# GuanLab/seekmer

Measured on AMD Instinct MI355X. Metric: paired reads/sec mapped+quantified, higher is better.
Workload: dtype u64+f64; 1 GPU; configs[1]: synthetic ~190k-tx index (stand-in for ENSEMBL GRCh38 cDNA), 10000000 2x100bp synthetic pairs per GPU, map+classes+EM to the reference stop rule; transcripts=190402, kmer_slots=134217728, units_per_gpu=10000000, read_len=100, paired=True, classes=851072, class_map_rows=4208693, parallelism=reads sharded x1, RCCL all-reduce f64[T] per EM step, rccl_ranks=0

## Files before the change

include/seekmer_hip.h:

```cpp
#ifndef SEEKMER_HIP_H
#define SEEKMER_HIP_H

#include <stddef.h>
#include <stdint.h>

#ifdef __cplusplus
extern "C" {
#endif

#define SKM_OK 0
#define SKM_ERR_ARG 1
#define SKM_ERR_HIP 2
#define SKM_ERR_NO_DEVICE 3
#define SKM_ERR_COLLISION 4
#define SKM_ERR_STATE 5
#define SKM_ERR_IO 6
#define SKM_ERR_UNDEFINED 7
#define SKM_ERR_COMM 8

#define SKM_KMER_SIZE 25
#define SKM_MAX_FRAGMENT_LENGTH 2000


const char *skm_last_error(void);
// ... 16 lines not shown
                     const char *sequences, int64_t n_bases,
                     const void *targets, int64_t n_targets,
                     int device, skm_index **out);
int skm_index_destroy(skm_index *index);
int skm_index_info(const skm_index *index, int64_t info[8]);
int skm_index_layout(const skm_index *index, int64_t layout[8]);
int skm_index_junctions(const skm_index *index, int32_t *succ, uint8_t *kept);
int skm_index_probe(const skm_index *index, int mode, const uint64_t *kmers, int64_t n, int32_t *entry,
                    int32_t *offset);
int skm_index_build_transcripts(skm_index *index, const double *lengths, int64_t n_tx);
int skm_index_transcript_bases(skm_index *index, char *bases_out, uint8_t *known_out);

typedef struct skm_mapper skm_mapper;
int skm_mapper_create(skm_index *index, skm_mapper **out);
int skm_mapper_destroy(skm_mapper *mapper);

int skm_mapper_map_batch(skm_mapper *mapper, const char *bases,
                         const int64_t *offsets, int64_t n_units, int paired);
int skm_mapper_map_batch_async(skm_mapper *mapper, const char *bases,
                               const int64_t *offsets, int64_t n_units, int paired,
                               int64_t first_unit);
int skm_mapper_map_batch_uniform_async(skm_mapper *mapper, const char *bases, int32_t read_len,
                                       int64_t n_units, int paired, int64_t first_unit);
int skm_mapper_sync(skm_mapper *mapper);
int skm_mapper_expect_units(skm_mapper *mapper, int64_t n_units);
#define SKM_PACKED_CUT (-1)
typedef struct skm_packed_reads {
    int32_t stream;
    int32_t code_words;
    int64_t first_read;
    int64_t n_reads;
    int64_t read_stride;
    int64_t uniform_len;
    const uint64_t *codes;
    const uint32_t *lengths;
    int64_t n_exceptions;
    const uint32_t *exception_reads;
    const uint32_t *exception_masks;
    const char *names;
    const int64_t *name_offsets;
} skm_packed_reads;
int skm_mapper_push_packed(skm_mapper *mapper, const skm_packed_reads *piece, int paired);
typedef int (*skm_packed_source)(void *context, skm_packed_reads *piece);
int skm_mapper_map_packed_source(skm_mapper *mapper, skm_packed_source next, void *context,
                                 int paired, int64_t *n_pieces);
int skm_mapper_map_batch_device(skm_mapper *mapper, const void *d_bases,
                                const void *d_offsets, int64_t n_units,
                                int paired, int32_t max_read_len);
int skm_mapper_last_batch(skm_mapper *mapper, int32_t *begin, int32_t *end,
                          int32_t *anchor_entry, int32_t *anchor_offset,
                          int32_t *counts, int32_t *entries,
                          int64_t cap_entries, int64_t *n_entries);
int skm_mapper_keep_spans(skm_mapper *mapper, int enable);
#define SKM_STRAND_NONE 0
#define SKM_STRAND_FR 1
#define SKM_STRAND_RF 2
int skm_mapper_set_strand(skm_mapper *mapper, int mode);
int skm_mapper_set_length_weights(skm_mapper *mapper, const double *p);
int skm_mapper_set_bias(skm_mapper *mapper, int enable);
int skm_mapper_bias_observed(skm_mapper *mapper, int64_t out[4096]);
int skm_mapper_summary(skm_mapper *mapper, int64_t summary[4]);
int skm_mapper_export(skm_mapper *mapper, int64_t *class_offsets,
                      int32_t *class_targets, int64_t *class_counts,
                      int64_t *first_seen, int64_t *fld);
int skm_mapper_merge(skm_mapper *mapper, int64_t n_classes,
                     const int64_t *class_offsets, const int32_t *class_targets,
                     const int64_t *class_counts, const int64_t *first_seen,
                     int64_t unaligned, const int64_t *fld);
typedef struct skm_device_table {
    int32_t device;
    int64_t n_classes, n_ids;
    const int64_t *class_start;
    const int64_t *class_len;
    const double *class_count;
    const uint64_t *first_seen;
    const int32_t *ids;
    int64_t unaligned, units, first_seen_bound;
    const uint64_t *fld;
} skm_device_table;
int skm_mapper_device_table(skm_mapper *mapper, skm_device_table *out);
int skm_mapper_merge_device(skm_mapper *mapper, const skm_device_table *table);
int skm_mapper_clear(skm_mapper *mapper);
int skm_mapper_reset(skm_mapper *mapper);
int skm_mapper_timing(skm_mapper *mapper, double stats[8]);
int skm_mapper_map_relaunches(skm_mapper *mapper, int64_t *count);
int skm_mapper_set_stats(skm_mapper *mapper, int enable);
int skm_mapper_access_stats(skm_mapper *mapper, int64_t out[48]);

typedef struct skm_sample_set skm_sample_set;
int skm_sample_set_create(skm_index *index, int paired, skm_sample_set **out);
int skm_sample_set_destroy(skm_sample_set *set);
int skm_sample_set_set_strand(skm_sample_set *set, int mode);
int skm_sample_set_set_length_weights(skm_sample_set *set, const double *p);
int skm_sample_set_add_packed(skm_sample_set *set, int64_t sample, int64_t first_unit,
                              const skm_packed_reads *mate1, const skm_packed_reads *mate2);
int skm_sample_set_add_batch(skm_sample_set *set, int64_t sample, int64_t first_unit,
                             const char *bases, const int64_t *offsets, int64_t n_units);
int skm_sample_set_sync(skm_sample_set *set);
int skm_sample_set_map_relaunches(skm_sample_set *set, int64_t *count);
int skm_sample_set_summary(skm_sample_set *set, int64_t cap_samples, int64_t *n_samples,
                           int64_t *summary);
int skm_sample_set_export(skm_sample_set *set, int64_t *sample_class_offsets,
                          int64_t *class_offsets, int32_t *class_targets, int64_t *class_counts,
                          int64_t *first_seen);
int skm_sample_set_histogram(skm_sample_set *set, int64_t *fld);
int skm_sample_set_keep_histograms(skm_sample_set *set, int enable);
// ... 192 lines not shown
```

seekmer_amd/_native.py:

```python
import ctypes
import os

_HERE = os.path.dirname(os.path.abspath(__file__))
HIP_LIB_PATH = os.environ.get('SKM_HIP_LIB') or os.path.join(_HERE, 'libseekmer_hip.so')
HOST_LIB_PATH = os.path.join(_HERE, 'libseekmer_host.so')

SKM_OK = 0
SKM_ERR_ARG = 1
SKM_ERR_HIP = 2
SKM_ERR_NO_DEVICE = 3
SKM_ERR_COLLISION = 4
SKM_ERR_STATE = 5
SKM_ERR_IO = 6
SKM_ERR_UNDEFINED = 7
SKM_ERR_COMM = 8

SKM_STRAND_NONE = 0
SKM_STRAND_FR = 1
SKM_STRAND_RF = 2

c_void_pp = ctypes.POINTER(ctypes.c_void_p)
c_i64p = ctypes.POINTER(ctypes.c_int64)
c_i32p = ctypes.POINTER(ctypes.c_int32)
c_f64p = ctypes.POINTER(ctypes.c_double)
# ... 9 lines not shown
                ('exception_reads', ctypes.c_void_p), ('exception_masks', ctypes.c_void_p),
                ('names', ctypes.c_void_p), ('name_offsets', ctypes.c_void_p)]


class DeviceTable(ctypes.Structure):
    _fields_ = [('device', ctypes.c_int32), ('n_classes', ctypes.c_int64), ('n_ids', ctypes.c_int64),
                ('class_start', ctypes.c_void_p), ('class_len', ctypes.c_void_p), ('class_count', ctypes.c_void_p),
                ('first_seen', ctypes.c_void_p), ('ids', ctypes.c_void_p), ('unaligned', ctypes.c_int64),
                ('units', ctypes.c_int64), ('first_seen_bound', ctypes.c_int64), ('fld', ctypes.c_void_p)]


HIP_SYMBOLS = {
    'skm_last_error': (ctypes.c_char_p, []),
    'skm_device_count': (ctypes.c_int, [ctypes.POINTER(ctypes.c_int)]),
    'skm_device_malloc': (ctypes.c_int, [ctypes.c_int, c_i64, c_void_pp]),
    'skm_device_free': (ctypes.c_int, [ctypes.c_int, ctypes.c_void_p]),
    'skm_device_upload': (ctypes.c_int, [ctypes.c_int, ctypes.c_void_p, ctypes.c_void_p, c_i64]),
    'skm_device_download': (ctypes.c_int, [ctypes.c_int, ctypes.c_void_p, ctypes.c_void_p, c_i64]),
    'skm_device_synchronize': (ctypes.c_int, [ctypes.c_int]),
    'skm_device_gather_ceiling': (ctypes.c_int, [ctypes.c_int, c_i64, ctypes.c_int, ctypes.c_int,
                                                 ctypes.c_int, c_f64p]),
    'skm_pinned_alloc': (ctypes.c_void_p, [ctypes.c_size_t]),
    'skm_pinned_free': (None, [ctypes.c_void_p]),
    'skm_pinned_set_device': (ctypes.c_int, [ctypes.c_int]),
    'skm_index_create': (ctypes.c_int, [ctypes.c_void_p, c_i64, ctypes.c_void_p, c_i64,
                                        ctypes.c_void_p, c_i64, ctypes.c_void_p, c_i64,
                                        ctypes.c_int, c_void_pp]),
    'skm_index_destroy': (ctypes.c_int, [ctypes.c_void_p]),
    'skm_index_info': (ctypes.c_int, [ctypes.c_void_p, c_i64p]),
    'skm_index_layout': (ctypes.c_int, [ctypes.c_void_p, c_i64p]),
    'skm_index_junctions': (ctypes.c_int, [ctypes.c_void_p, c_i32p, ctypes.c_void_p]),
    'skm_index_probe': (ctypes.c_int, [ctypes.c_void_p, ctypes.c_int, c_u64p, c_i64, c_i32p, c_i32p]),
    'skm_index_build_transcripts': (ctypes.c_int, [ctypes.c_void_p, c_f64p, c_i64]),
    'skm_index_transcript_bases': (ctypes.c_int, [ctypes.c_void_p, ctypes.c_void_p, ctypes.c_void_p]),
    'skm_mapper_create': (ctypes.c_int, [ctypes.c_void_p, c_void_pp]),
    'skm_mapper_destroy': (ctypes.c_int, [ctypes.c_void_p]),
    'skm_mapper_map_batch': (ctypes.c_int, [ctypes.c_void_p, ctypes.c_void_p, c_i64p, c_i64,
                                            ctypes.c_int]),
    'skm_mapper_map_batch_async': (ctypes.c_int, [ctypes.c_void_p, ctypes.c_void_p, c_i64p, c_i64,
                                                  ctypes.c_int, c_i64]),
    'skm_mapper_map_batch_uniform_async': (ctypes.c_int, [ctypes.c_void_p, ctypes.c_void_p, ctypes.c_int32, c_i64,
                                                          ctypes.c_int, c_i64]),
    'skm_mapper_sync': (ctypes.c_int, [ctypes.c_void_p]),
    'skm_mapper_expect_units': (ctypes.c_int, [ctypes.c_void_p, c_i64]),
    'skm_mapper_push_packed': (ctypes.c_int, [ctypes.c_void_p, ctypes.POINTER(PackedReads), ctypes.c_int]),
    'skm_mapper_map_packed_source': (ctypes.c_int, [ctypes.c_void_p, ctypes.c_void_p, ctypes.c_void_p, ctypes.c_int,
                                                    c_i64p]),
    'skm_mapper_map_batch_device': (ctypes.c_int, [ctypes.c_void_p, ctypes.c_void_p,
                                                   ctypes.c_void_p, c_i64, ctypes.c_int,
                                                   ctypes.c_int32]),
    'skm_mapper_last_batch': (ctypes.c_int, [ctypes.c_void_p, c_i32p, c_i32p, c_i32p, c_i32p,
                                             c_i32p, c_i32p, c_i64, c_i64p]),
    'skm_mapper_keep_spans': (ctypes.c_int, [ctypes.c_void_p, ctypes.c_int]),
    'skm_mapper_set_strand': (ctypes.c_int, [ctypes.c_void_p, ctypes.c_int]),
    'skm_mapper_set_length_weights': (ctypes.c_int, [ctypes.c_void_p, c_f64p]),
    'skm_mapper_set_bias': (ctypes.c_int, [ctypes.c_void_p, ctypes.c_int]),
    'skm_mapper_bias_observed': (ctypes.c_int, [ctypes.c_void_p, c_i64p]),
    'skm_mapper_summary': (ctypes.c_int, [ctypes.c_void_p, c_i64p]),
    'skm_mapper_export': (ctypes.c_int, [ctypes.c_void_p, c_i64p, c_i32p, c_i64p, c_i64p, c_i64p]),
    'skm_mapper_merge': (ctypes.c_int, [ctypes.c_void_p, c_i64, c_i64p, c_i32p, c_i64p, c_i64p,
                                        c_i64, c_i64p]),
    'skm_mapper_device_table': (ctypes.c_int, [ctypes.c_void_p, ctypes.POINTER(DeviceTable)]),
    'skm_mapper_merge_device': (ctypes.c_int, [ctypes.c_void_p, ctypes.POINTER(DeviceTable)]),
    'skm_mapper_clear': (ctypes.c_int, [ctypes.c_void_p]),
    'skm_mapper_reset': (ctypes.c_int, [ctypes.c_void_p]),
    'skm_mapper_timing': (ctypes.c_int, [ctypes.c_void_p, c_f64p]),
    'skm_mapper_map_relaunches': (ctypes.c_int, [ctypes.c_void_p, c_i64p]),
    'skm_sample_set_map_relaunches': (ctypes.c_int, [ctypes.c_void_p, c_i64p]),
    'skm_mapper_set_stats': (ctypes.c_int, [ctypes.c_void_p, ctypes.c_int]),
    'skm_mapper_access_stats': (ctypes.c_int, [ctypes.c_void_p, c_i64p]),
    'skm_effective_lengths': (ctypes.c_int, [ctypes.c_int, c_i64p, c_f64p, c_i64, c_f64p]),
    'skm_effective_lengths_many': (ctypes.c_int, [ctypes.c_int, c_i64, c_i64p, c_f64p, c_i64, c_f64p]),
    'skm_effective_lengths_weights': (ctypes.c_int, [ctypes.c_int, c_i64, c_f64p, c_f64p, c_i64, c_f64p]),
    'skm_bias_correct': (ctypes.c_int, [ctypes.c_void_p, ctypes.c_int, c_i64p, c_f64p, c_f64p, c_i64, c_f64p, c_f64p, c_f64p]),
    'skm_bias_correct_many': (ctypes.c_int, [ctypes.c_void_p, ctypes.c_int, c_i64, c_i64p, c_f64p, c_f64p, c_i64, c_f64p,
                                             c_f64p, c_f64p]),
    'skm_sample_set_create': (ctypes.c_int, [ctypes.c_void_p, ctypes.c_int, c_void_pp]),
    'skm_sample_set_destroy': (ctypes.c_int, [ctypes.c_void_p]),
    'skm_sample_set_set_strand': (ctypes.c_int, [ctypes.c_void_p, ctypes.c_int]),
    'skm_sample_set_set_length_weights': (ctypes.c_int, [ctypes.c_void_p, c_f64p]),
    'skm_sample_set_add_packed': (ctypes.c_int, [ctypes.c_void_p, c_i64, c_i64, ctypes.POINTER(PackedReads),
                                                 ctypes.POINTER(PackedReads)]),
    'skm_sample_set_add_batch': (ctypes.c_int, [ctypes.c_void_p, c_i64, c_i64, ctypes.c_void_p, c_i64p, c_i64]),
    'skm_sample_set_sync': (ctypes.c_int, [ctypes.c_void_p]),
    'skm_sample_set_summary': (ctypes.c_int, [ctypes.c_void_p, c_i64, c_i64p, c_i64p]),
    'skm_sample_set_export': (ctypes.c_int, [ctypes.c_void_p, c_i64p, c_i64p, c_i32p, c_i64p, c_i64p]),
    'skm_sample_set_histogram': (ctypes.c_int, [ctypes.c_void_p, c_i64p]),
    'skm_sample_set_keep_histograms': (ctypes.c_int, [ctypes.c_void_p, ctypes.c_int]),
    'skm_sample_set_histograms': (ctypes.c_int, [ctypes.c_void_p, c_i64, c_i64p]),
    'skm_sample_set_keep_bias': (ctypes.c_int, [ctypes.c_void_p, ctypes.c_int]),
    'skm_sample_set_bias_observed': (ctypes.c_int, [ctypes.c_void_p, c_i64, c_i64p]),
    'skm_sample_set_keep_umis': (ctypes.c_int, [ctypes.c_void_p, ctypes.c_int]),
    'skm_sample_set_add_packed_umis': (ctypes.c_int, [ctypes.c_void_p, c_i64, c_i64, ctypes.POINTER(PackedReads),
                                                      ctypes.POINTER(PackedReads), c_u32p]),
    'skm_sample_set_umi_removed': (ctypes.c_int, [ctypes.c_void_p, c_i64, c_i64p]),
    'skm_umi_windows': (ctypes.c_int, [ctypes.c_int, ctypes.POINTER(PackedReads), ctypes.c_int, ctypes.c_int, c_i32p, c_u32p,
                                       c_i64p]),
    'skm_sample_set_plan': (ctypes.c_int, [c_i64, c_i32p, c_i64p, c_i64, c_i64, c_i64p, c_i64p, c_i64p, c_i32p]),
    'skm_sample_set_split': (ctypes.c_int, [c_i64, c_i64p, c_i64p, c_i32p, c_i64, c_i64, c_i64p, c_i32p, c_i64p, c_i64p,
                                            c_i64p]),
    'skm_gene_sums': (ctypes.c_int, [ctypes.c_int, c_i64, c_i64, c_i64, c_i32p, c_f64p, c_f64p]),
    'skm_gene_unique_counts': (ctypes.c_int, [ctypes.c_int, c_i64, c_i64p, c_i32p, c_i64p, c_i32p, c_i64, c_i64, c_i64,
                                              c_i32p, c_i64p, c_i64p]),
    'skm_mapper_gene_counts': (ctypes.c_int, [ctypes.c_void_p, c_i64, c_i64, c_i32p, c_i64p, c_i64p]),
    'skm_sample_set_gene_counts': (ctypes.c_int, [ctypes.c_void_p, c_i64, c_i64, c_i32p, c_i64, c_i64p, c_i64p]),
    'skm_barcodes_create': (ctypes.c_int, [ctypes.c_int, ctypes.c_char_p, c_i64, ctypes.c_int, c_void_pp]),
# ... 171 lines not shown
```

seekmer_amd/csrc/skm_abi.hip:

```cpp
#include "skm_abi.h"
#include "skm_bias.h"
#include "skm_bias_weights.h"

#include <dlfcn.h>
#include <algorithm>
#include <cmath>
#include <cstdarg>
#include <cstdio>
#include <cstdlib>
#include <cstring>
#include <chrono>
#include <condition_variable>
#include <atomic>
#include <deque>
#include <functional>
#include <map>
#include <memory>
#include <unordered_map>
#include <mutex>
#include <thread>
#include <numeric>
#include <string>
#include <utility>
#include <vector>
// ... 7 lines not shown
    DevIndex d{};
    DevMem kmers, contigs, seq2, buckets, edge_kmers, signatures;
    int64_t n_slots = 0, bytes = 0;
    int64_t layout[8] = {0};
    int cu_count = 256;
    std::atomic<int> holders{1};
    std::mutex pool_mu;
    std::vector<PoolContig> pool_contigs;
    std::vector<Coord> pool_targets;
    bool pool_built = false;
    TxPool pool{};
    DevMem pool_codes, pool_known, pool_tx_word, pool_tx_len, pool_tx_windows;
    std::vector<int64_t> pool_tx_base;
    std::vector<int32_t> pool_windows;
};

struct skm_mapper {
    explicit skm_mapper(skm_index *index) : ix(index) { index->holders.fetch_add(1); }
    ~skm_mapper();
    Own<skm_index *, skm_index_destroy> ix;
    PoolStream stream;
    Event ev[4];
    std::mutex mu;
    ClassTable t{};
    DBuf<ClassSlot> slots;
    DBuf<int32_t> arena;
    DBuf<int64_t> class_list;
    DBuf<unsigned long long> counters;
    DBuf<int> error;
    DBuf<uint8_t> bases;
    DBuf<int64_t> offsets;
    DBuf<uint32_t> records;
    DBuf<int32_t> workspace;
    DBuf<int32_t> unit_begin, unit_end, rec_unit;
    DBuf<Coord> unit_anchor;
    DBuf<int64_t> unit_slot;
    DBuf<unsigned long long> rec_tuple;
    HostPinned pinned;
    DBuf<uint64_t> rec_key;
    bool keep_spans = false, last_spans = false;
    int strand = SKM_STRAND_NONE;
    bool bias = false;
    DBuf<unsigned long long> bias_observed;
    DBuf<double> length_weights;
    bool use_length_weights = false;
    DBuf<int32_t> unit_entries;
    DBuf<unsigned long long> batch_ctl;
    int grid_blocks = 0;
    int64_t expected_units = 0;
    bool packed_sized = false;
    int64_t units_done = 0;
    int64_t first_seen_bound = 0;
    int64_t last_units = 0, last_ids = 0;
    int64_t host_classes = 0, host_arena_used = 0;
    bool host_totals_valid = false;
    unsigned long long host_units = 0, host_unaligned = 0;
    int want_stats = 0;
    double t_pack_ns = 0, t_map_ns = 0, t_class_ns = 0, batches = 0;
    double t_em_ns = 0, em_iters = 0;
    bool test_class_slots = false;
    int64_t deferred_grows = 0;
    int test_map_blocks = 0;
    int64_t map_relaunches = 0;
    unsigned long long stats_total[48] = {0};
    struct Lane {
        DBuf<uint8_t> bases;
        DBuf<int64_t> offsets;
        Stream stream;
        bool busy = false;
    };
    static constexpr int N_LANES = 3;
    Lane lanes[N_LANES];
    struct Job { int lane; int64_t n_units; int paired; int64_t offset_base; int64_t first_unit; uint64_t ticket; };
    std::mutex q_mu;
    std::condition_variable q_cv;
    std::condition_variable done_cv;
    std::deque<Job> jobs;
    std::thread worker;
    bool worker_started = false, stop = false;
    uint64_t next_ticket = 1, done_ticket = 0;
    int job_error = SKM_OK;
    uint64_t job_error_ticket = 0;
    std::string job_error_msg;
    DBuf<unsigned long long> scan_out;
    struct Piece {
        int64_t first = 0, n = 0;
        int64_t origin = 0;
        int cw = 1;
        int64_t uniform_len = -1;
        std::shared_ptr<char> block;
        uint64_t *codes = nullptr;
        uint32_t *lengths = nullptr;
        uint32_t *exc_reads_dev = nullptr, *exc_masks = nullptr;
        std::vector<uint32_t> exc_reads;
        bool in_job = false;
    };
    std::deque<Piece> pending[2];
    Stream packed_stream;
    int packed_paired = -1;
    int packed_flush = 0;
    int packed_waiters = 0;
    int64_t packed_max_pending = 8LL << 30;
    bool packed_busy = false;
    int64_t packed_dropped = 0;
    std::shared_ptr<std::atomic<int64_t>> packed_bytes = std::make_shared<std::atomic<int64_t>>(0);
    int vote[8] = {1, 1, 1, 1, 1, 1, 1, 0};
// ... 691 lines not shown
    drain.dismiss();
    m->slots = std::move(new_slots);
    bind_table(m, need);
    return SKM_OK;
}

int table_reserve_for_sample(skm_mapper *m, int64_t sample_units)
{
    const double expect = (double)m->host_classes + (double)std::min<int64_t>(sample_units, 1LL << 29) / 8.0 + 1024.0;
    uint64_t want = 1 << 16;
    while ((double)want * 0.5 < expect && want < (1ULL << 26)) want <<= 1;
    if (!m->test_class_slots) SKM_TRY(table_grow(m, want, 0));
    SKM_TRY(m->class_list.ensure((size_t)(expect + 1024.0), true, m->stream));
    SKM_TRY(m->arena.ensure((size_t)(m->host_arena_used + (int64_t)(expect * 6.0) + 1024), true, m->stream));
    bind_table(m, m->t.slot_mask + 1);
    return SKM_OK;
}

int table_reserve(skm_mapper *m, int64_t n_units)
{
    const double expect = (double)m->host_classes + (double)n_units / 8.0 + 1024.0;
    uint64_t want = 1 << 16;
    while ((double)want * 0.5 < expect) want <<= 1;
    if (!m->test_class_slots) SKM_TRY(table_grow(m, want, 0));
    SKM_TRY(m->class_list.ensure((size_t)(m->host_classes + n_units + 1024), true, m->stream));
    bind_table(m, m->t.slot_mask + 1);
    return SKM_OK;
}

int read_error(skm_mapper *m)
{
    int err = 0;
    HIP_TRY(hipMemcpyAsync(&err, m->error.p, sizeof(int), hipMemcpyDeviceToHost, m->stream));
    HIP_TRY(hipStreamSynchronize(m->stream));
    if (err == SKM_ERR_COLLISION)
        return fail(SKM_ERR_COLLISION, "two different class tuples share a 64-bit key");
    if (err) return fail(err, "class table kernel reported error %d", err);
    return SKM_OK;
}

typedef std::function<int(uint32_t *, int, int)> RecordStage;
typedef std::function<int(const MapBatch &)> BatchStage;
int map_batch_resident(skm_mapper *m, const uint8_t *d_bases, const int64_t *d_offsets,
                       int64_t n_units, int paired, int max_len, int64_t first_unit = -1,
                       const RecordStage *fill_records = nullptr, const SampleSalt *salt = nullptr,
                       unsigned long long *sample_bias_rows = nullptr, const BatchStage *collapse = nullptr)
{
    const int64_t unit_base = first_unit >= 0 ? first_unit : m->units_done;
    skm_index *ix = m->ix;
    const int64_t n_reads = paired ? 2 * n_units : n_units;
    const int words = (max_len + 31) / 32 + 1;
    m->last_units = n_units;
    m->last_ids = 0;
    if (n_units == 0) return SKM_OK;

    const int record_words = ((3 * words + 1 + 15) / 16) * 16;
    SKM_TRY(m->records.ensure((size_t)n_reads * record_words + 16));
    if (n_units >= (1LL << 31)) return fail(SKM_ERR_ARG, "more than 2^31 - 1 units in one batch");
    if (m->keep_spans) {
        SKM_TRY(m->unit_begin.ensure(n_units));
        SKM_TRY(m->unit_end.ensure(n_units));
        SKM_TRY(m->unit_anchor.ensure(n_units));
    }
    m->last_spans = m->keep_spans;
    SKM_TRY(m->rec_unit.ensure(n_units));
    SKM_TRY(m->rec_tuple.ensure(n_units));
    SKM_TRY(m->unit_slot.ensure(n_units));
    SKM_TRY(m->rec_key.ensure(n_units));

    SKM_TRY(m->batch_ctl.ensure(BC_WORDS));

    constexpr int64_t CONTEXTS = MAP_CONTEXTS;
    int64_t blocks = std::min<int64_t>((n_units + CONTEXTS - 1) / CONTEXTS, (int64_t)ix->cu_count * MAP_BLOCKS_PER_CU);
    if (m->test_map_blocks) blocks = std::min<int64_t>(blocks, m->test_map_blocks);
    const int64_t ext_words = std::max<int64_t>(0, (ix->d.max_target_count + 63) / 64 - 1);
    SKM_TRY(m->workspace.ensure((size_t)(blocks * CONTEXTS * 4 * ext_words * 2 + 16)));
    m->grid_blocks = (int)blocks;
    {
        const int64_t per_block = (n_units + blocks - 1) / blocks;
        if (per_block * (paired ? 2 : 1) * (int64_t)record_words * 4 >= (1LL << 32))
            return fail(SKM_ERR_ARG, "batch of %lld units with %d-base reads is too large for one launch",
                        (long long)n_units, max_len);
    }
    SKM_TRY(m->unit_entries.ensure((size_t)n_units * 8 + (size_t)blocks * (MAP_THREADS / 64) * MAP_ARENA_CHUNK + 4096));

    MapBatch b{};
    b.records = m->records.p;
    b.n_units = n_units;
    b.words_per_read = words;
    b.record_words = record_words;
    b.paired = paired;
    b.workspace = m->workspace.p;
    b.unit_begin = m->unit_begin.p;
    b.unit_end = m->unit_end.p;
    b.unit_anchor = m->unit_anchor.p;
    b.keep_spans = m->keep_spans ? 1 : 0;
    b.rec_unit = m->rec_unit.p;
    b.rec_tuple = m->rec_tuple.p;
    b.rec_key = m->rec_key.p;
    b.ids_cursor = m->batch_ctl.p + BC_IDS;
    b.fld = m->batch_ctl.p + BC_FLD;
    b.stats = m->batch_ctl.p + BC_STATS;
    for (int i = 0; i < 8; ++i) b.vote[i] = m->vote[i];

    HIP_TRY(hipEventRecord(m->ev[0], m->stream));
    if (fill_records) SKM_TRY((*fill_records)(m->records.p, words, record_words));
    else launch_pack_reads(d_bases, d_offsets, n_reads, words, record_words, m->records.p, m->stream);
    HIP_TRY(hipGetLastError());
    HIP_TRY(hipEventRecord(m->ev[1], m->stream));
    unsigned long long ids = 0;
// ... 762 lines not shown
                                     int32_t *entries, int64_t cap_entries, int64_t *n_entries)
{
    if (!m) return fail(SKM_ERR_ARG, "NULL mapper");
    SKM_TRY(wait_jobs(m, 0, false));
    std::lock_guard<std::mutex> lock(m->mu);
    SKM_TRY(set_device(m->ix->device));
    const int64_t n = m->last_units;
    if (n_entries) *n_entries = 0;
    if (n == 0) return SKM_OK;
    if ((begin || end || anchor_entry || anchor_offset) && !m->last_spans)
        return fail(SKM_ERR_STATE, "the spans of the last batch were not kept: call skm_mapper_keep_spans(mapper, 1) before mapping");
    if (begin) HIP_TRY(hipMemcpy(begin, m->unit_begin.p, n * 4, hipMemcpyDeviceToHost));
    if (end) HIP_TRY(hipMemcpy(end, m->unit_end.p, n * 4, hipMemcpyDeviceToHost));
    if (anchor_entry || anchor_offset) {
        std::vector<Coord> a(n);
        HIP_TRY(hipMemcpy(a.data(), m->unit_anchor.p, n * sizeof(Coord), hipMemcpyDeviceToHost));
        for (int64_t i = 0; i < n; ++i) {
            if (anchor_entry) anchor_entry[i] = a[i].entry;
            if (anchor_offset) anchor_offset[i] = a[i].offset;
        }
    }
    if (!counts && !entries && !n_entries) return SKM_OK;
    std::vector<int32_t> unit(n);
    std::vector<unsigned long long> tuple(n);
    HIP_TRY(hipMemcpy(unit.data(), m->rec_unit.p, n * 4, hipMemcpyDeviceToHost));
    HIP_TRY(hipMemcpy(tuple.data(), m->rec_tuple.p, n * 8, hipMemcpyDeviceToHost));
    std::vector<int32_t> cnt(n, 0);
    std::vector<int64_t> off(n, 0);
    std::vector<char> seen(n, 0);
    for (int64_t r = 0; r < n; ++r) {
        const int64_t u = unit[r];
        if (u < 0 || u >= n || seen[u]) return fail(SKM_ERR_STATE, "record %lld names unit %lld", (long long)r, (long long)u);
        seen[u] = 1;
        cnt[u] = (int32_t)(tuple[r] >> 40);
        off[u] = (int64_t)(tuple[r] & ((1ULL << 40) - 1));
    }
    if (counts) memcpy(counts, cnt.data(), n * 4);
    if (n_entries) {
        int64_t total = 0;
        for (int64_t u = 0; u < n; ++u) total += cnt[u];
        *n_entries = total;
    }
    if (entries) {
        std::vector<int32_t> raw((size_t)std::max<int64_t>(m->last_ids, 1));
        if (m->last_ids)
            HIP_TRY(hipMemcpy(raw.data(), m->unit_entries.p, (size_t)m->last_ids * 4, hipMemcpyDeviceToHost));
        int64_t pos = 0;
        for (int64_t u = 0; u < n; ++u) {
            for (int i = 0; i < cnt[u]; ++i)
                if (pos + i < cap_entries) entries[pos + i] = raw[off[u] + i];
            pos += cnt[u];
        }
    }
    return SKM_OK;
}

extern "C" int skm_mapper_keep_spans(skm_mapper *m, int enable)
{
    if (!m) return fail(SKM_ERR_ARG, "NULL mapper");
    (void)wait_jobs(m, 0, false);
    std::lock_guard<std::mutex> lock(m->mu);
    m->keep_spans = enable != 0;
    return SKM_OK;
}

extern "C" int skm_mapper_set_strand(skm_mapper *m, int mode)
{
    if (!m) return fail(SKM_ERR_ARG, "NULL mapper");
    if (mode != SKM_STRAND_NONE && mode != SKM_STRAND_FR && mode != SKM_STRAND_RF)
        return fail(SKM_ERR_ARG, "unknown strand mode %d", mode);
    (void)wait_jobs(m, 0, false);
    bool queued;
    {
        std::lock_guard<std::mutex> hold(m->q_mu);
        queued = !m->jobs.empty() || m->packed_busy || !m->pending[0].empty() || !m->pending[1].empty();
    }
    std::lock_guard<std::mutex> lock(m->mu);
    if (queued || m->units_done != 0)
        return fail(SKM_ERR_STATE, "the strand mode can only change on an empty mapper (new, or after "
                                   "skm_mapper_reset / skm_mapper_clear)");
    m->strand = mode;
    return SKM_OK;
}

extern "C" int skm_mapper_set_bias(skm_mapper *m, int enable)
{
    if (!m) return fail(SKM_ERR_ARG, "NULL mapper");
    (void)wait_jobs(m, 0, false);
    bool queued;
    {
        std::lock_guard<std::mutex> hold(m->q_mu);
        queued = !m->jobs.empty() || m->packed_busy || !m->pending[0].empty() || !m->pending[1].empty();
    }
    std::lock_guard<std::mutex> lock(m->mu);
    if (queued || m->units_done != 0)
        return fail(SKM_ERR_STATE, "hexamer counting can only change on an empty mapper (new, or after "
                                   "skm_mapper_reset / skm_mapper_clear)");
    if (enable) {
        SKM_TRY(set_device(m->ix->device));
        SKM_TRY(m->bias_observed.ensure(BIAS_BINS));
        HIP_TRY(hipMemsetAsync(m->bias_observed.p, 0, BIAS_BINS * sizeof(unsigned long long), m->stream));
        HIP_TRY(hipStreamSynchronize(m->stream));
    }
    m->bias = enable != 0;
    return SKM_OK;
}
// ... 213 lines not shown
                                  (const unsigned long long *)table->first_seen, m->stream);
        HIP_TRY(hipGetLastError());
        SKM_TRY(read_error(m));
    }
    launch_class_add_totals(m->t, (unsigned long long)table->unaligned, (unsigned long long)table->units,
                            (const unsigned long long *)table->fld, m->stream);
    HIP_TRY(hipGetLastError());
    unsigned long long ctr[8];
    HIP_TRY(hipMemcpyAsync(ctr, m->counters.p, sizeof(ctr), hipMemcpyDeviceToHost, m->stream));
    HIP_TRY(hipStreamSynchronize(m->stream));
    m->host_arena_used = (int64_t)ctr[CTR_ARENA];
    m->host_classes = (int64_t)ctr[CTR_CLASSES];
    m->host_units = ctr[CTR_UNITS];
    m->host_unaligned = ctr[CTR_UNALIGNED];
    m->host_totals_valid = true;
    m->units_done += table->units;
    m->first_seen_bound = std::max(m->first_seen_bound, std::max(table->first_seen_bound, m->units_done));
    return SKM_OK;
}

extern "C" int skm_mapper_clear(skm_mapper *m)
{
    if (!m) return fail(SKM_ERR_ARG, "NULL mapper");
    (void)wait_jobs(m, 0, true);
    {
        std::lock_guard<std::mutex> hold(m->q_mu);
        packed_drop_all(m);
    }
    std::lock_guard<std::mutex> lock(m->mu);
    SKM_TRY(set_device(m->ix->device));
    std::vector<unsigned long long> fld(MAX_FRAGMENT_LENGTH);
    HIP_TRY(hipMemcpy(fld.data(), m->counters.p + CTR_FLD, MAX_FRAGMENT_LENGTH * 8, hipMemcpyDeviceToHost));
    SKM_TRY(table_reset(m, m->t.slot_mask + 1));
    HIP_TRY(hipMemcpyAsync(m->counters.p + CTR_FLD, fld.data(), MAX_FRAGMENT_LENGTH * 8, hipMemcpyHostToDevice, m->stream));
    HIP_TRY(hipStreamSynchronize(m->stream));
    return SKM_OK;
}

extern "C" int skm_mapper_reset(skm_mapper *m)
{
    if (!m) return fail(SKM_ERR_ARG, "NULL mapper");
    (void)wait_jobs(m, 0, true);
    {
        std::lock_guard<std::mutex> hold(m->q_mu);
        packed_drop_all(m);
    }
    std::lock_guard<std::mutex> lock(m->mu);
    SKM_TRY(set_device(m->ix->device));
    SKM_TRY(table_reset(m, m->t.slot_mask + 1));
    if (m->bias) HIP_TRY(hipMemsetAsync(m->bias_observed.p, 0, BIAS_BINS * sizeof(unsigned long long), m->stream));
    HIP_TRY(hipStreamSynchronize(m->stream));
    m->last_units = 0;
    m->last_ids = 0;
    return SKM_OK;
}

extern "C" int skm_mapper_timing(skm_mapper *m, double stats[8])
{
    if (!m || !stats) return fail(SKM_ERR_ARG, "NULL argument");
    (void)wait_jobs(m, 0, false);
    std::lock_guard<std::mutex> lock(m->mu);
    stats[0] = m->t_pack_ns; stats[1] = m->t_map_ns; stats[2] = m->t_class_ns;
    stats[3] = m->batches; stats[4] = (double)m->units_done;
    stats[5] = m->t_em_ns; stats[6] = m->em_iters; stats[7] = (double)m->deferred_grows;
    return SKM_OK;
}

extern "C" int skm_mapper_map_relaunches(skm_mapper *m, int64_t *count)
{
    if (!m || !count) return fail(SKM_ERR_ARG, "NULL argument");
    (void)wait_jobs(m, 0, false);
    std::lock_guard<std::mutex> lock(m->mu);
    *count = m->map_relaunches;
    return SKM_OK;
}

extern "C" int skm_mapper_access_stats(skm_mapper *m, int64_t out[48])
{
    if (!m || !out) return fail(SKM_ERR_ARG, "NULL argument");
    (void)wait_jobs(m, 0, false);
    std::lock_guard<std::mutex> lock(m->mu);
    for (int i = 0; i < 48; ++i) out[i] = (int64_t)m->stats_total[i];
    return SKM_OK;
}

extern "C" int skm_mapper_set_stats(skm_mapper *m, int enable)
{
    if (!m) return fail(SKM_ERR_ARG, "NULL mapper");
    (void)wait_jobs(m, 0, false);
    std::lock_guard<std::mutex> lock(m->mu);
    m->want_stats = enable == 2 ? 2 : (enable != 0 ? 1 : 0);
    for (auto &v : m->stats_total) v = 0;
    return SKM_OK;
}

namespace {

struct SetChunk {
    std::deque<skm_mapper::Piece> pieces[2];
    std::shared_ptr<char> ascii;
    const uint8_t *bases = nullptr;
    const int64_t *offsets = nullptr;
    int64_t origin = 0;
    int max_len = 0;
    std::shared_ptr<uint32_t> umis;
    int64_t umi_origin = 0;
// ... 2501 lines not shown
```

seekmer_amd/csrc/skm_kernels.h:

```cpp
#pragma once
#include "skm_device.h"

namespace skm {

struct MapBatch {
    const uint32_t *records;
    int64_t n_units;
    int32_t words_per_read;
    int32_t record_words;
    int32_t paired;
    int32_t *workspace;
    int32_t *rec_unit;
    uint64_t *rec_key;
    unsigned long long *rec_tuple;
    int32_t keep_spans;
    int32_t *unit_begin, *unit_end;
    Coord *unit_anchor;
    int32_t *unit_entries;
    int64_t ids_capacity;
    int32_t ids_chunk;
    unsigned long long *ids_cursor;
    unsigned long long *fld;
    unsigned long long *stats;
    int32_t vote[8];
};

#ifndef SKM_MAP_THREADS
#define SKM_MAP_THREADS 256
#endif
#ifndef SKM_MAP_WAVES_PER_EU
#define SKM_MAP_WAVES_PER_EU 4
#endif
constexpr int MAP_THREADS = SKM_MAP_THREADS;
constexpr int MAP_BLOCKS_PER_CU = 4;
#ifndef SKM_MAP_CONTEXTS
#define SKM_MAP_CONTEXTS 480
#endif
constexpr int MAP_CONTEXTS = SKM_MAP_CONTEXTS;
constexpr int MAP_ARENA_CHUNK = 2048;

void launch_pack_reads(const uint8_t *bases, const int64_t *offsets, int64_t n_reads,
                       int words_per_read, int record_words, uint32_t *records, hipStream_t stream);
void launch_unpack_reads(const uint64_t *codes, int64_t stride, int code_words, const uint32_t *lengths,
                         uint32_t uniform_len, int64_t n_reads, int words_per_read, uint32_t *dst,
                         int64_t dst_stride, int *error, hipStream_t stream);
void launch_unpack_exceptions(const uint32_t *exc_reads, const uint32_t *exc_masks, int64_t n_exceptions,
                              int code_words, int64_t first_read, int words_per_read, uint32_t *dst,
                              int64_t dst_stride, hipStream_t stream);
void launch_offsets_scan(int64_t *offsets, int64_t n_reads, int64_t base, unsigned long long *out,
                         hipStream_t stream);
void launch_offsets_uniform(int64_t *offsets, int64_t n_reads, int64_t read_len, hipStream_t stream);
void launch_bucket_build(const DevIndex &ix, uint64_t n_slots, DevBucket *buckets, uint32_t bucket_mask,
                         uint32_t bucket_shift, unsigned long long *report, hipStream_t stream);
void launch_signature_build(const DevBucket *buckets, uint64_t n_buckets, uint64_t *signatures, uint32_t shift,
                            hipStream_t stream);
void launch_successor_build(const DevIndex &ix, DevContig *records, int64_t n_contigs, int force_lookup,
                            hipStream_t stream);
void launch_index_probe(const DevIndex &ix, int mode, const uint64_t *kmers, int64_t n, int32_t *entry, int32_t *offset,
                        hipStream_t stream);
void launch_map_units(const DevIndex &ix, const MapBatch &b, int grid_blocks, int stats,
                      hipStream_t stream);
void launch_pack_sequences(const char *bases, int64_t n_bases, uint64_t *seq2, int64_t n_words,
                           hipStream_t stream);
void launch_strand_filter(const MapBatch &b, int mode, hipStream_t stream);

template <class T>
__host__ __device__ __forceinline__ int64_t segment_find(const T *first, int64_t n, int64_t unit)
{
    int64_t lo = 0, hi = n;
    while (hi - lo > 1) {
        const int64_t mid = (lo + hi) >> 1;
        if ((int64_t)first[mid] <= unit) lo = mid; else hi = mid;
    }
    return lo;
}
constexpr uint64_t SAMPLE_KEY_STEP = 0xD6E8FEB86659FD93ULL;
__host__ __device__ __forceinline__ uint64_t sample_key(uint64_t key, uint32_t sample) { return key + sample * SAMPLE_KEY_STEP; }
constexpr int SAMPLE_LAUNCH_SEGMENTS = 2048;
struct SampleSalt {
    const int32_t *seg_first;
    const int32_t *seg_sample;
    int32_t n_segments;
};
void launch_sample_salt(const MapBatch &b, const SampleSalt &salt, int *error, hipStream_t stream);
void launch_sample_fld(const int32_t *unit_begin, const int32_t *unit_end, int64_t n_units, const SampleSalt &salt,
                       unsigned long long *hist, hipStream_t stream);
void launch_sample_bias(const MapBatch &b, const SampleSalt &salt, unsigned long long *rows, hipStream_t stream);
void launch_sample_assign(const int64_t *log_global, const int64_t *log_local, const int32_t *log_sample,
                          int64_t n_segments, const unsigned long long *cls_first_seen, int64_t n_classes,
                          int32_t *cls_sample, int64_t *cls_local, hipStream_t stream);

void launch_gather_probe(const void *table, uint64_t n_slots, int blocks, int per_lane, int chain,
                         unsigned long long *sink, hipStream_t stream);

struct alignas(32) ClassSlot {
// ... 420 lines not shown
```

seekmer_amd/csrc/skm_map.hip:

```cpp
#include "../../include/seekmer_hip.h"
#include "skm_device.h"
#include "skm_kernels.h"

namespace skm {

struct __attribute__((packed, aligned(1))) Bytes16 { uint32_t w[4]; };

__device__ __forceinline__ void pack_byte(uint32_t ch, int i, uint64_t &codes, uint32_t &acgt)
{
    codes |= (uint64_t)two_bit_encode(ch) << (62 - 2 * i);
    const bool up = ch == 'A' || ch == 'C' || ch == 'G' || ch == 'T';
    acgt |= (uint32_t)up << (31 - i);
}

__device__ __forceinline__ void pack_dword(uint32_t w, int first, int n, uint64_t &codes, uint32_t &acgt)
{
    const int cnt = n - first;
    if (cnt <= 0) return;
    const uint32_t keep = cnt >= 4 ? 0xffffffffu : ((1u << (8 * cnt)) - 1u);
    const uint32_t up = w & 0xDFDFDFDFu;
    const uint32_t idx = (up >> 1) & 0x03030303u;
    const uint32_t expect = __builtin_amdgcn_perm(0u, 0x47544341u, idx);
    const uint32_t t = up ^ expect;
    uint32_t valid = ~(((t & 0x7F7F7F7Fu) + 0x7F7F7F7Fu) | t | 0x7F7F7F7Fu);
// ... 21 lines not shown
    const uint32_t a = __builtin_amdgcn_perm(p0, p1, 0x07030000u);
    const uint32_t b = __builtin_amdgcn_perm(p2, p3, 0x00000703u);
    return __builtin_amdgcn_perm(a, b, 0x07060100u);
}

__global__ void __launch_bounds__(256)
pack_reads_kernel(const uint8_t *__restrict__ bases, const int64_t *__restrict__ offsets,
                  int64_t n_reads, int words_per_read, int record_words, uint32_t *__restrict__ records)
{
    const int64_t total = n_reads * (int64_t)words_per_read;
    const int64_t end_of_bases = offsets[n_reads];
    const bool shifting = (words_per_read & (words_per_read - 1)) == 0;
    const int shift = __builtin_ctz((unsigned)words_per_read);
    for (int64_t g = blockIdx.x * (int64_t)blockDim.x + threadIdx.x; g < total;
         g += (int64_t)gridDim.x * blockDim.x) {
        const int64_t r = shifting ? g >> shift
                                   : total <= 0xffffffffLL ? (int64_t)((uint32_t)g / (uint32_t)words_per_read)
                                                           : g / words_per_read;
        const int w = (int)(g - r * words_per_read);
        const int64_t begin = offsets[r];
        const int len = (int)(offsets[r + 1] - begin);
        uint64_t c = 0;
        uint32_t m = 0;
        const int first = w * 32;
        if (first < len) {
            const int n = min(32, len - first);
            const int64_t at = begin + first;
            if (at + 32 <= end_of_bases) {
                const Bytes16 lo = *reinterpret_cast<const Bytes16 *>(bases + at);
                const Bytes16 hi = *reinterpret_cast<const Bytes16 *>(bases + at + 16);
                uint32_t bad = 0;
                const uint32_t first16 = top_bytes(pack_dword_plain(lo.w[0], bad), pack_dword_plain(lo.w[1], bad),
                                                   pack_dword_plain(lo.w[2], bad), pack_dword_plain(lo.w[3], bad));
                const uint32_t last16 = top_bytes(pack_dword_plain(hi.w[0], bad), pack_dword_plain(hi.w[1], bad),
                                                  pack_dword_plain(hi.w[2], bad), pack_dword_plain(hi.w[3], bad));
                if (bad == 0) {
                    m = n >= 32 ? 0xffffffffu : ~(0xffffffffu >> n);
                    c = (((uint64_t)first16 << 32) | last16) & (n >= 32 ? ~0ULL : ~(~0ULL >> (2 * n)));
                } else {
#pragma unroll
                    for (int d = 0; d < 4; ++d) pack_dword(lo.w[d], 4 * d, n, c, m);
#pragma unroll
                    for (int d = 0; d < 4; ++d) pack_dword(hi.w[d], 16 + 4 * d, n, c, m);
                }
            } else {
                for (int i = 0; i < n; ++i) pack_byte(bases[at + i], i, c, m);
            }
        }
        uint32_t *rec = records + r * (int64_t)record_words;
        reinterpret_cast<uint64_t *>(rec)[w] = c;
        rec[2 * words_per_read + w] = m;
        if (w == 0) rec[3 * words_per_read] = (uint32_t)len;
        for (int k = 3 * words_per_read + 1 + w; k < record_words; k += words_per_read) rec[k] = 0;
    }
}

__global__ void __launch_bounds__(256)
unpack_reads_kernel(const uint64_t *__restrict__ codes, int64_t stride, int code_words,
                    const uint32_t *__restrict__ lengths, uint32_t uniform_len, int64_t n_reads,
                    int words_per_read, uint32_t *__restrict__ dst, int64_t dst_stride, int *error)
{
    const int64_t total = n_reads * (int64_t)words_per_read;
    for (int64_t g = blockIdx.x * (int64_t)blockDim.x + threadIdx.x; g < total;
         g += (int64_t)gridDim.x * blockDim.x) {
        const int64_t r = total <= 0xffffffffLL ? (int64_t)((uint32_t)g / (uint32_t)words_per_read)
                                                : g / words_per_read;
        const int w = (int)(g - r * words_per_read);
        uint32_t len = lengths ? lengths[r] : uniform_len;
        if (len > 32u * (uint32_t)code_words) {
            len = 32u * (uint32_t)code_words;
            if (w == 0) atomicExch(error, SKM_ERR_ARG);
        }
        const uint64_t c = w < code_words ? codes[r * stride + w] : 0;
        const int n = (int)len - 32 * w;
        const uint32_t m = n >= 32 ? 0xffffffffu : (n <= 0 ? 0u : ~(0xffffffffu >> n));
        uint32_t *rec = dst + r * dst_stride;
        reinterpret_cast<uint64_t *>(rec)[w] = c;
        rec[2 * words_per_read + w] = m;
        if (w == 0) rec[3 * words_per_read] = len;
    }
}

__global__ void __launch_bounds__(256)
unpack_exceptions_kernel(const uint32_t *__restrict__ exc_reads, const uint32_t *__restrict__ exc_masks,
                         int64_t n_exceptions, int code_words, int64_t first_read, int words_per_read,
                         uint32_t *__restrict__ dst, int64_t dst_stride)
{
    const int64_t total = n_exceptions * (int64_t)code_words;
    for (int64_t g = blockIdx.x * (int64_t)blockDim.x + threadIdx.x; g < total;
         g += (int64_t)gridDim.x * blockDim.x) {
        const int64_t e = g / code_words;
        const int w = (int)(g - e * code_words);
        const int64_t r = (int64_t)exc_reads[e] - first_read;
        if (w < words_per_read) dst[r * dst_stride + 2 * words_per_read + w] = exc_masks[g];
    }
}

__global__ void __launch_bounds__(256)
offsets_scan_kernel(int64_t *offsets, int64_t n_reads, int64_t base, unsigned long long *out)
{
    long long longest = 0;
    unsigned long long descents = 0;
    for (int64_t r = blockIdx.x * (int64_t)blockDim.x + threadIdx.x; r < n_reads;
         r += (int64_t)gridDim.x * blockDim.x) {
        const long long len = offsets[r + 1] - offsets[r];
        if (len < 0) ++descents;
// ... 1310 lines not shown
    hipLaunchKernelGGL(bucket_fill_kernel, dim3(4096), dim3(256), 0, stream, ix.kmers, n_slots, filling,
                       bucket_mask, bucket_shift, report);
    hipLaunchKernelGGL(bucket_pack_kernel, dim3(4096), dim3(256), 0, stream, filling, (uint64_t)bucket_mask + 1);
    hipLaunchKernelGGL(probe_check_kernel, dim3(4096), dim3(256), 0, stream, ix, n_slots, report);
}

void launch_signature_build(const DevBucket *buckets, uint64_t n_buckets, uint64_t *signatures, uint32_t shift,
                            hipStream_t stream)
{
    hipLaunchKernelGGL(signature_build_kernel, dim3(4096), dim3(256), 0, stream, buckets, n_buckets,
                       reinterpret_cast<unsigned long long *>(signatures), shift);
}

void launch_successor_build(const DevIndex &ix, DevContig *records, int64_t n_contigs, int force_lookup,
                            hipStream_t stream)
{
    hipLaunchKernelGGL(successor_build_kernel, dim3(2048), dim3(256), 0, stream, ix, records, n_contigs, force_lookup);
}

void launch_index_probe(const DevIndex &ix, int mode, const uint64_t *kmers, int64_t n, int32_t *entry, int32_t *offset,
                        hipStream_t stream)
{
    if (n <= 0) return;
    int64_t blocks = (n + 255) / 256;
    if (blocks > 4096) blocks = 4096;
    hipLaunchKernelGGL(index_probe_kernel, dim3((unsigned)blocks), dim3(256), 0, stream, ix, mode, kmers, n, entry, offset);
}

void launch_offsets_scan(int64_t *offsets, int64_t n_reads, int64_t base, unsigned long long *out,
                         hipStream_t stream)
{
    if (n_reads <= 0) return;
    int64_t blocks = (n_reads + 255) / 256;
    if (blocks > 2048) blocks = 2048;
    hipLaunchKernelGGL(offsets_scan_kernel, dim3((unsigned)blocks), dim3(256), 0, stream, offsets, n_reads, base, out);
    if (base != 0)
        hipLaunchKernelGGL(offsets_rebase_kernel, dim3((unsigned)blocks), dim3(256), 0, stream, offsets,
                           n_reads + 1, base);
}

void launch_offsets_uniform(int64_t *offsets, int64_t n_reads, int64_t read_len, hipStream_t stream)
{
    int64_t blocks = (n_reads + 1 + 255) / 256;
    if (blocks > 2048) blocks = 2048;
    hipLaunchKernelGGL(offsets_uniform_kernel, dim3((unsigned)blocks), dim3(256), 0, stream, offsets, n_reads + 1,
                       read_len);
}

void launch_pack_reads(const uint8_t *bases, const int64_t *offsets, int64_t n_reads,
                       int words_per_read, int record_words, uint32_t *records, hipStream_t stream)
{
    const int64_t total = n_reads * (int64_t)words_per_read;
    if (total == 0) return;
    int64_t blocks = (total + 255) / 256;
    if (blocks > 256 * 32) blocks = 256 * 32;
    hipLaunchKernelGGL(pack_reads_kernel, dim3((unsigned)blocks), dim3(256), 0, stream,
                       bases, offsets, n_reads, words_per_read, record_words, records);
}

void launch_unpack_reads(const uint64_t *codes, int64_t stride, int code_words, const uint32_t *lengths,
                         uint32_t uniform_len, int64_t n_reads, int words_per_read, uint32_t *dst,
                         int64_t dst_stride, int *error, hipStream_t stream)
{
    const int64_t total = n_reads * (int64_t)words_per_read;
    if (total == 0) return;
    int64_t blocks = (total + 255) / 256;
    if (blocks > 256 * 32) blocks = 256 * 32;
    hipLaunchKernelGGL(unpack_reads_kernel, dim3((unsigned)blocks), dim3(256), 0, stream, codes, stride, code_words,
                       lengths, uniform_len, n_reads, words_per_read, dst, dst_stride, error);
}

void launch_unpack_exceptions(const uint32_t *exc_reads, const uint32_t *exc_masks, int64_t n_exceptions,
                              int code_words, int64_t first_read, int words_per_read, uint32_t *dst,
                              int64_t dst_stride, hipStream_t stream)
{
    const int64_t total = n_exceptions * (int64_t)code_words;
    if (total == 0) return;
    int64_t blocks = (total + 255) / 256;
    if (blocks > 256 * 32) blocks = 256 * 32;
    hipLaunchKernelGGL(unpack_exceptions_kernel, dim3((unsigned)blocks), dim3(256), 0, stream, exc_reads, exc_masks,
                       n_exceptions, code_words, first_read, words_per_read, dst, dst_stride);
}

void launch_map_units(const DevIndex &ix, const MapBatch &b, int grid_blocks, int stats,
                      hipStream_t stream)
{
    if (b.n_units == 0) return;
    if (stats == 2 && ix.buckets)
        hipLaunchKernelGGL((map_units_kernel<true, true>), dim3(grid_blocks), dim3(MAP_THREADS), 0, stream, ix, b);
    else if (stats)
        hipLaunchKernelGGL((map_units_kernel<true, false>), dim3(grid_blocks), dim3(MAP_THREADS), 0, stream, ix, b);
    else if (ix.buckets)
        hipLaunchKernelGGL((map_units_kernel<false, true>), dim3(grid_blocks), dim3(MAP_THREADS), 0, stream, ix, b);
    else
        hipLaunchKernelGGL((map_units_kernel<false, false>), dim3(grid_blocks), dim3(MAP_THREADS), 0, stream, ix, b);
}

void warm_code_map()
{
    hipFuncAttributes attributes;
    (void)hipFuncGetAttributes(&attributes, reinterpret_cast<const void *>(&map_units_kernel<false, true>));
    (void)hipFuncGetAttributes(&attributes, reinterpret_cast<const void *>(&unpack_reads_kernel));
}

}
```

Measured before the change: 1.018 billion pairs/s.

## Stage read packing through LDS with coalesced vector loads and stores

Adds a pack_reads_staged_kernel. Each block loads a contiguous span of base bytes as 16-byte vectors with nontemporal loads, encodes them into 2-bit code and flag streams in LDS, then writes whole 16-byte record chunks using bit-aligned windows. This replaces per-read, per-word gathers with coalesced global traffic. The cost is more complex indexing and extra LDS use. It also adds copy_records and pack_stage_reads helpers for testing and inspection.

```diff
diff --git a/include/seekmer_hip.h b/include/seekmer_hip.h
--- a/include/seekmer_hip.h
+++ b/include/seekmer_hip.h
@@ -92,6 +92,9 @@
                           int32_t *counts, int32_t *entries,
                           int64_t cap_entries, int64_t *n_entries);
 int skm_mapper_keep_spans(skm_mapper *mapper, int enable);
+int skm_mapper_copy_records(skm_mapper *mapper, int64_t first_read, int64_t n_reads, uint32_t *out,
+                            int32_t *record_words, int32_t *words_per_read);
+int skm_pack_stage_reads(int32_t words_per_read, int32_t *reads_per_block);
 #define SKM_STRAND_NONE 0
 #define SKM_STRAND_FR 1
 #define SKM_STRAND_RF 2
diff --git a/seekmer_amd/_native.py b/seekmer_amd/_native.py
--- a/seekmer_amd/_native.py
+++ b/seekmer_amd/_native.py
@@ -85,6 +85,8 @@
     'skm_mapper_last_batch': (ctypes.c_int, [ctypes.c_void_p, c_i32p, c_i32p, c_i32p, c_i32p,
                                              c_i32p, c_i32p, c_i64, c_i64p]),
     'skm_mapper_keep_spans': (ctypes.c_int, [ctypes.c_void_p, ctypes.c_int]),
+    'skm_mapper_copy_records': (ctypes.c_int, [ctypes.c_void_p, c_i64, c_i64, c_u32p, c_i32p, c_i32p]),
+    'skm_pack_stage_reads': (ctypes.c_int, [ctypes.c_int32, c_i32p]),
     'skm_mapper_set_strand': (ctypes.c_int, [ctypes.c_void_p, ctypes.c_int]),
     'skm_mapper_set_length_weights': (ctypes.c_int, [ctypes.c_void_p, c_f64p]),
     'skm_mapper_set_bias': (ctypes.c_int, [ctypes.c_void_p, ctypes.c_int]),
diff --git a/seekmer_amd/csrc/skm_abi.hip b/seekmer_amd/csrc/skm_abi.hip
--- a/seekmer_amd/csrc/skm_abi.hip
+++ b/seekmer_amd/csrc/skm_abi.hip
@@ -83,6 +83,8 @@
     int64_t units_done = 0;
     int64_t first_seen_bound = 0;
     int64_t last_units = 0, last_ids = 0;
+    int64_t last_reads = 0;
+    int last_words = 0, last_record_words = 0;
     int64_t host_classes = 0, host_arena_used = 0;
     bool host_totals_valid = false;
     unsigned long long host_units = 0, host_unaligned = 0;
@@ -880,10 +882,14 @@
     const int words = (max_len + 31) / 32 + 1;
     m->last_units = n_units;
     m->last_ids = 0;
+    m->last_reads = 0;
     if (n_units == 0) return SKM_OK;
 
     const int record_words = ((3 * words + 1 + 15) / 16) * 16;
     SKM_TRY(m->records.ensure((size_t)n_reads * record_words + 16));
+    m->last_reads = n_reads;
+    m->last_words = words;
+    m->last_record_words = record_words;
     if (n_units >= (1LL << 31)) return fail(SKM_ERR_ARG, "more than 2^31 - 1 units in one batch");
     if (m->keep_spans) {
         SKM_TRY(m->unit_begin.ensure(n_units));
@@ -1752,6 +1758,34 @@
             pos += cnt[u];
         }
     }
+    return SKM_OK;
+}
+
+extern "C" int skm_mapper_copy_records(skm_mapper *m, int64_t first_read, int64_t n_reads, uint32_t *out,
+                                       int32_t *record_words, int32_t *words_per_read)
+{
+    if (!m) return fail(SKM_ERR_ARG, "NULL mapper");
+    SKM_TRY(wait_jobs(m, 0, false));
+    std::lock_guard<std::mutex> lock(m->mu);
+    SKM_TRY(set_device(m->ix->device));
+    if (m->last_reads == 0) return fail(SKM_ERR_STATE, "no batch has been mapped since the handle was made or reset");
+    if (first_read < 0 || n_reads < 0 || first_read > m->last_reads || n_reads > m->last_reads - first_read)
+        return fail(SKM_ERR_ARG, "reads %lld .. +%lld of a batch of %lld", (long long)first_read, (long long)n_reads,
+                    (long long)m->last_reads);
+    if (record_words) *record_words = m->last_record_words;
+    if (words_per_read) *words_per_read = m->last_words;
+    if (out && n_reads) {
+        HIP_TRY(hipStreamSynchronize(m->stream));
+        HIP_TRY(hipMemcpy(out, m->records.p + first_read * (int64_t)m->last_record_words,
+                          (size_t)n_reads * m->last_record_words * 4, hipMemcpyDeviceToHost));
+    }
+    return SKM_OK;
+}
+
+extern "C" int skm_pack_stage_reads(int32_t words_per_read, int32_t *reads_per_block)
+{
+    if (words_per_read < 1 || !reads_per_block) return fail(SKM_ERR_ARG, "bad argument");
+    *reads_per_block = pack_stage_reads(words_per_read);
     return SKM_OK;
 }
 
@@ -2071,6 +2105,7 @@
     HIP_TRY(hipStreamSynchronize(m->stream));
     m->last_units = 0;
     m->last_ids = 0;
+    m->last_reads = 0;
     return SKM_OK;
 }
 
diff --git a/seekmer_amd/csrc/skm_kernels.h b/seekmer_amd/csrc/skm_kernels.h
--- a/seekmer_amd/csrc/skm_kernels.h
+++ b/seekmer_amd/csrc/skm_kernels.h
@@ -41,6 +41,7 @@
 
 void launch_pack_reads(const uint8_t *bases, const int64_t *offsets, int64_t n_reads,
                        int words_per_read, int record_words, uint32_t *records, hipStream_t stream);
+int pack_stage_reads(int words_per_read);
 void launch_unpack_reads(const uint64_t *codes, int64_t stride, int code_words, const uint32_t *lengths,
                          uint32_t uniform_len, int64_t n_reads, int words_per_read, uint32_t *dst,
                          int64_t dst_stride, int *error, hipStream_t stream);
diff --git a/seekmer_amd/csrc/skm_map.hip b/seekmer_amd/csrc/skm_map.hip
--- a/seekmer_amd/csrc/skm_map.hip
+++ b/seekmer_amd/csrc/skm_map.hip
@@ -97,6 +97,159 @@
         rec[2 * words_per_read + w] = m;
         if (w == 0) rec[3 * words_per_read] = (uint32_t)len;
         for (int k = 3 * words_per_read + 1 + w; k < record_words; k += words_per_read) rec[k] = 0;
+    }
+}
+
+constexpr int PACK_STAGE_BYTES = 8192;
+constexpr int PACK_STAGE_MAX_READS = 128;
+constexpr int PACK_STAGE_MIN_READS = 16;
+constexpr int PACK_STAGE_LOADS = 4;
+constexpr int PACK_STAGE_THREADS = 256;
+static_assert(PACK_STAGE_MAX_READS < PACK_STAGE_THREADS, "a lane per read of the block, and one more");
+typedef uint32_t PackVec4 __attribute__((ext_vector_type(4)));
+#ifndef SKM_PACK_NONTEMPORAL
+#define SKM_PACK_NONTEMPORAL 3
+#endif
+#if SKM_PACK_NONTEMPORAL & 1
+#define PACK_LOAD(p) __builtin_nontemporal_load(p)
+#else
+#define PACK_LOAD(p) (*(p))
+#endif
+#if SKM_PACK_NONTEMPORAL & 2
+#define PACK_STORE(v, p) __builtin_nontemporal_store(v, p)
+#else
+#define PACK_STORE(v, p) (*(p) = (v))
+#endif
+
+struct PackStage {
+    int reads_per_block;
+    int code_words;
+    int flag_words;
+    uint32_t chunk_magic;
+    size_t lds_bytes() const { return 4 * (size_t)(reads_per_block + 1 + code_words + flag_words); }
+};
+static PackStage pack_stage(int words_per_read, int record_words)
+{
+    PackStage s{};
+    const int base_words = words_per_read > 1 ? words_per_read - 1 : 1;
+    int reads = PACK_STAGE_BYTES / (12 * base_words);
+    if (reads > PACK_STAGE_MAX_READS) reads = PACK_STAGE_MAX_READS;
+#if defined(SKM_PACK_STAGED) && !SKM_PACK_STAGED
+    reads = 0;
+#endif
+    if (reads < PACK_STAGE_MIN_READS) return s;
+    s.reads_per_block = reads;
+    s.code_words = reads * 2 * base_words + 5;
+    s.flag_words = reads * base_words + 4;
+    s.chunk_magic = 0xffffffffu / (uint32_t)(record_words / 4) + 1u;
+    return s;
+}
+int pack_stage_reads(int words_per_read)
+{
+    return pack_stage(words_per_read, 16).reads_per_block;
+}
+
+__device__ __forceinline__ uint32_t stream_window(const uint32_t *stream, uint32_t word, uint32_t shift, uint32_t last)
+{
+    const uint32_t i = min(word, last);
+    const uint32_t a = stream[i], b = stream[i + 1];
+    return shift ? __builtin_amdgcn_alignbit(a, b, 32u - shift) : a;
+}
+
+__global__ void __launch_bounds__(PACK_STAGE_THREADS)
+pack_reads_staged_kernel(const uint8_t *__restrict__ bases, const int64_t *__restrict__ offsets,
+                         int64_t n_reads, int words_per_read, int record_words, PackStage stage,
+                         uint32_t *__restrict__ records)
+{
+    extern __shared__ uint32_t pack_lds[];
+    int32_t *at = reinterpret_cast<int32_t *>(pack_lds);
+    uint32_t *codes = pack_lds + stage.reads_per_block + 1;
+    uint32_t *flags = codes + stage.code_words;
+
+    const int64_t r0 = blockIdx.x * (int64_t)stage.reads_per_block;
+    const int reads = n_reads - r0 < stage.reads_per_block ? (int)(n_reads - r0) : stage.reads_per_block;
+    const int64_t first_of_bases = offsets[0], end_of_bases = offsets[n_reads];
+    const int64_t span_begin = offsets[r0], span_end = offsets[r0 + reads];
+    const int head = (int)(reinterpret_cast<uintptr_t>(bases + span_begin) & 15u);
+    const int64_t chunk0 = span_begin - head;
+    const int64_t span_chunks = span_end > span_begin ? (span_end - chunk0 + 15) >> 4 : 0;
+    const int n_chunks = span_chunks < stage.code_words - 4 ? (int)span_chunks : stage.code_words - 4;
+    const int64_t whole_from = first_of_bases > chunk0 ? (first_of_bases - chunk0 + 15) >> 4 : 0;
+    const int64_t whole_to = (end_of_bases - chunk0) >> 4;
+    const int first_whole = whole_from < n_chunks ? (int)whole_from : n_chunks;
+    const int end_whole = whole_to < n_chunks ? (whole_to > 0 ? (int)whole_to : 0) : n_chunks;
+
+    const int64_t my_offset = (int)threadIdx.x <= reads ? offsets[r0 + threadIdx.x] : 0;
+    for (int k0 = threadIdx.x; k0 < n_chunks; k0 += PACK_STAGE_LOADS * PACK_STAGE_THREADS) {
+        PackVec4 v[PACK_STAGE_LOADS];
+        bool whole[PACK_STAGE_LOADS];
+#pragma unroll
+        for (int u = 0; u < PACK_STAGE_LOADS; ++u) {
+            const int k = k0 + PACK_STAGE_THREADS * u;
+            whole[u] = k >= first_whole && k < end_whole;
+            if (whole[u]) v[u] = PACK_LOAD(reinterpret_cast<const PackVec4 *>(bases + chunk0) + k);
+        }
+#pragma unroll
+        for (int u = 0; u < PACK_STAGE_LOADS; ++u) {
+            const int k = k0 + PACK_STAGE_THREADS * u;
+            if (k >= n_chunks) break;
+            uint32_t w[4] = {v[u].x, v[u].y, v[u].z, v[u].w};
+            if (!whole[u]) {
+                const int64_t pos = chunk0 + 16 * (int64_t)k;
+#pragma unroll
+                for (int d = 0; d < 4; ++d) {
+                    w[d] = 0;
+#pragma unroll
+                    for (int i = 0; i < 4; ++i) {
+                        const int64_t p = pos + 4 * d + i;
+                        if (p >= first_of_bases && p < end_of_bases) w[d] |= (uint32_t)bases[p] << (8 * i);
+                    }
+                }
+            }
+            uint32_t bad = 0;
+            uint32_t code = top_bytes(pack_dword_plain(w[0], bad), pack_dword_plain(w[1], bad),
+                                      pack_dword_plain(w[2], bad), pack_dword_plain(w[3], bad));
+            uint32_t flag = 0xffffu;
+            if (bad != 0) {
+                uint64_t c = 0;
+                uint32_t m = 0;
+#pragma unroll
+                for (int d = 0; d < 4; ++d) pack_dword(w[d], 4 * d, 16, c, m);
+                code = (uint32_t)(c >> 32);
+                flag = m >> 16;
+            }
+            codes[k] = code;
+            reinterpret_cast<uint16_t *>(flags)[k ^ 1] = (uint16_t)flag;
+        }
+    }
+    if ((int)threadIdx.x <= reads) at[threadIdx.x] = (int32_t)(my_offset - chunk0);
+    __syncthreads();
+
+    const int chunks_per_record = record_words >> 2;
+    const int total = reads * chunks_per_record;
+    const uint32_t last_code = (uint32_t)stage.code_words - 2u, last_flag = (uint32_t)stage.flag_words - 2u;
+    PackVec4 *out = reinterpret_cast<PackVec4 *>(records + r0 * (int64_t)record_words);
+    for (int i = threadIdx.x; i < total; i += PACK_STAGE_THREADS) {
+        const int r = (int)__umulhi((uint32_t)i, stage.chunk_magic);
+        const int first_word = 4 * (i - r * chunks_per_record);
+        const int begin = at[r];
+        const int len = at[r + 1] - begin;
+        const uint32_t code_at = (uint32_t)begin >> 4, code_shift = 2u * ((uint32_t)begin & 15u);
+        const uint32_t flag_at = (uint32_t)begin >> 5, flag_shift = (uint32_t)begin & 31u;
+        uint32_t v[4];
+#pragma unroll
+        for (int t = 0; t < 4; ++t) {
+            const int j = first_word + t;
+            const bool is_code = j < 2 * words_per_read;
+            const int k = is_code ? j ^ 1 : j - 2 * words_per_read;
+            const int bits = min(max(is_code ? 2 * len - 32 * k : j < 3 * words_per_read ? len - 32 * k : 0, 0), 32);
+            v[t] = stream_window(is_code ? codes : flags, (is_code ? code_at : flag_at) + (uint32_t)k,
+                                 is_code ? code_shift : flag_shift, is_code ? last_code : last_flag);
+            v[t] = bits >= 32 ? v[t] : v[t] & ~(0xffffffffu >> bits);
+            if (j == 3 * words_per_read) v[t] = (uint32_t)len;
+        }
+        const PackVec4 piece = {v[0], v[1], v[2], v[3]};
+        PACK_STORE(piece, out + i);
     }
 }
 
@@ -1513,6 +1666,13 @@
 {
     const int64_t total = n_reads * (int64_t)words_per_read;
     if (total == 0) return;
+    const PackStage stage = pack_stage(words_per_read, record_words);
+    const int64_t staged_blocks = stage.reads_per_block ? (n_reads + stage.reads_per_block - 1) / stage.reads_per_block : 0;
+    if (stage.reads_per_block && staged_blocks <= 0x7fffffffLL) {
+        hipLaunchKernelGGL(pack_reads_staged_kernel, dim3((unsigned)staged_blocks), dim3(PACK_STAGE_THREADS), stage.lds_bytes(), stream,
+                           bases, offsets, n_reads, words_per_read, record_words, stage, records);
+        return;
+    }
     int64_t blocks = (total + 255) / 256;
     if (blocks > 256 * 32) blocks = 256 * 32;
     hipLaunchKernelGGL(pack_reads_kernel, dim3((unsigned)blocks), dim3(256), 0, stream,
```

After: 1.034 billion pairs/s (median of 6 runs). 1.02x the previous value.
